# Ichoran/dbce-video-cpp

Measured on AMD Instinct MI355X. Metric: frames/s + raw-pixel GB/s, 4096x3072 U8 encode+decode round-trip, higher is better.
Workload: dtype u8

## Files before the change

### dbde-video-cpp_amd/csrc/dbde_kernels.hip

```cpp
#include "dbde_kernels.h"

#include "dbde_bits.h"
#include "dbde_device.h"


namespace dbde {

#ifndef DBDE_DIAG_LATE
#define DBDE_DIAG_LATE 34
#endif
#ifdef DBDE_DIAG
#define SF_DECL uint64_t sfd[10] = {0, 0, 0, 0, 0, 0, 0, 0, 0, 0}
#define SF_MARK(i) do { if (threadIdx.x == 0) sfd[i] = wall_clock64(); } while (0)
#define SF_DRAIN() asm volatile("s_waitcnt vmcnt(0) lgkmcnt(0)" ::: "memory")
#define SF_FLUSH(diag, last)                                                                          \
    do {                                                                                              \
        if (threadIdx.x == 0 && (diag)) {                                                             \
            atomicMax(&(diag)[0], ~(unsigned long long)sfd[0]);                                       \
            for (int i_ = 1; i_ < 10; i_++) atomicAdd(&(diag)[i_], (unsigned long long)sfd[i_]);      \
            atomicAdd(&(diag)[10], 1ull);                                                             \
            atomicMax(&(diag)[11], (unsigned long long)sfd[last]);                                    \
            atomicMax(&(diag)[12], (unsigned long long)sfd[0]);                                       \
            atomicAdd(&(diag)[13], (unsigned long long)sfd[0]);                                       \
        }                                                                                             \
    } while (0)
#else
#define SF_DECL
#define SF_MARK(i)
#define SF_DRAIN()
#define SF_FLUSH(diag, last)
#endif

typedef uint32_t u32x4_t __attribute__((ext_vector_type(4)));

typedef unsigned long long u64a;


__device__ __forceinline__ uint64_t load_u64_any(const uint8_t *p) {
    uint64_t v;
    __builtin_memcpy(&v, p, 8);
    return v;
}
__device__ __forceinline__ void store_u64_any(uint8_t *p, uint64_t v) { __builtin_memcpy(p, &v, 8); }
__device__ __forceinline__ void store_u32_bytes(uint8_t *p, uint32_t v) {
    p[0] = (uint8_t)v; p[1] = (uint8_t)(v >> 8); p[2] = (uint8_t)(v >> 16); p[3] = (uint8_t)(v >> 24);
}
__device__ __forceinline__ uint32_t load_u32_bytes(const uint8_t *p) {
    return (uint32_t)p[0] | ((uint32_t)p[1] << 8) | ((uint32_t)p[2] << 16) | ((uint32_t)p[3] << 24);
}
__device__ __forceinline__ uint64_t load_u64_bytes(const uint8_t *p) {
    return (uint64_t)load_u32_bytes(p) | ((uint64_t)load_u32_bytes(p + 4) << 32);
}

template <int NW = 4>
__device__ __forceinline__ uint32_t block_scan_incl(uint32_t v, uint32_t *s_wave_tot, int lane, int wave,
                                                    uint32_t &block_total) {
    uint32_t incl = v;
#pragma unroll
    for (int o = 1; o < 64; o <<= 1) {
        uint32_t n = __shfl_up(incl, o, 64);
        if (lane >= o) incl += n;
    }
    if (lane == 63) s_wave_tot[wave] = incl;
    __syncthreads();
    uint32_t base = 0, tot = 0;
#pragma unroll
    for (int k = 0; k < NW; k++) {
        const uint32_t tk = s_wave_tot[k];
        base += k < wave ? tk : 0u;
        tot += tk;
    }
    block_total = tot;
    return base + incl;
}

__device__ __forceinline__ uint32_t swz8(uint32_t slot) { return slot ^ ((slot >> 3) & 7u); }
__device__ __forceinline__ uint32_t swz16(uint32_t slot) { return slot ^ ((slot >> 4) & 15u); }
__device__ __forceinline__ uint32_t swzq8(uint32_t q) { return (swz8(q >> 1) << 1) | (q & 1u); }
__device__ __forceinline__ uint32_t swzq16(uint32_t q) { return (swz16(q >> 1) << 1) | (q & 1u); }

__device__ __forceinline__ uint32_t depth_bytes_bad(uint32_t x, uint32_t min_bytes) {
    return min_bytes == 1u ? ((x & 0xF0F0F0F0u) | (((x & 0x0F0F0F0Fu) + 0x77777777u) & 0x80808080u))
                           : ((x & 0xE0E0E0E0u) | (((x & 0x1F1F1F1Fu) + 0x6F6F6F6Fu) & 0x80808080u));
}

__device__ __forceinline__ uint64_t f64_to_u64_x86(double v) {
    const double two63 = 9223372036854775808.0;
    bool high = v >= two63;
    double a = high ? v - two63 : v;
    uint64_t r;
    if (a >= -two63 && a < two63) r = (uint64_t)(long long)a;
    else r = 0x8000000000000000ull;
    return high ? (r ^ 0x8000000000000000ull) : r;
}

__device__ __forceinline__ bool in_extent(uint64_t off, uint64_t len, uint64_t extent) {
    return off <= extent && len <= extent - off;
}

__device__ __forceinline__ uint32_t div_magic(uint32_t n, uint32_t d, uint32_t m, uint32_t &rem) {
    uint32_t q = __umulhi(n, m);
    uint32_t r = n - q * d;
    const bool fix = r >= d;
    q += fix ? 1u : 0u;
    r -= fix ? d : 0u;
    rem = r;
    return q;
}


__device__ __forceinline__ void load_tile_generic(const uint8_t *img, int W, int H, uint32_t w, uint32_t t,
                                                  uint32_t (&v)[16]) {
    uint32_t ty = t / w, tx = t - ty * w;
    int x0 = 8 * (int)tx;
    int rm = W - x0 < 8 ? W - x0 : 8;
#pragma unroll
    for (int r = 0; r < 8; r++) {
        int yy = 8 * (int)ty + r;
        yy = yy < H ? yy : H - 1;
        const uint8_t *row = img + (size_t)yy * (size_t)W + x0;
        uint64_t q;
        if (rm == 8) {
            q = load_u64_any(row);
        } else if (W >= 8) {
            q = load_u64_any(row + rm - 8) >> (8 * (8 - rm));
            const uint64_t last = (q >> (8 * (rm - 1))) & 0xFFull;
            q |= (last * 0x0101010101010101ull) << (8 * rm);
        } else {
            q = 0;
#pragma unroll
            for (int k = 0; k < 8; k++) {
                int kk = k < rm ? k : rm - 1;
                q |= (uint64_t)row[kk] << (8 * k);
            }
        }
        v[2 * r] = (uint32_t)q;
        v[2 * r + 1] = (uint32_t)(q >> 32);
    }
}

template <bool ALIGNED_OUT, int PIX = 1>
__device__ __forceinline__ void write_frame_fields(const EncParams &p, uint32_t f, uint32_t cf, uint32_t inf_incl,
                                                     uint32_t frame_start_glob) {
    const uint64_t meta = 32ull + (uint64_t)(1 + PIX) * p.T;
    const uint64_t frame_base = p.slot_stride ? (uint64_t)f * p.slot_stride
                                              : (uint64_t)f * meta + 8ull * (uint64_t)frame_start_glob;
    uint8_t *fb = p.out + frame_base;
    if (cf == 0u) {
        const uint64_t index = p.indices ? p.indices[f] : p.first_index + f;
        const uint64_t el = p.elapsed_ns ? p.elapsed_ns[f] : 0ull;
        const uint64_t elbits = (uint64_t)__double_as_longlong(__ull2double_rn(el));
        if (ALIGNED_OUT) {
            uint32_t *h = reinterpret_cast<uint32_t *>(fb);
            h[0] = 2u;
            h[1] = (uint32_t)index; h[2] = (uint32_t)(index >> 32);
            h[3] = (uint32_t)elbits; h[4] = (uint32_t)(elbits >> 32);
// ... 1087 lines not shown
    SF_FLUSH(p.diag, 9);
#endif
}

hipError_t launch_encode_small(const EncParams &p, bool fast_in, bool aligned_out, hipStream_t s) {
    dim3 block(kEncThreads), grid(p.n_chunks);
    switch (in_mode_of(p, fast_in) * 2 + (aligned_out ? 1 : 0)) {
        case kInFast * 2 + 1: hipLaunchKernelGGL((encode_small_kernel<kInFast, true>), grid, block, 0, s, p); break;
        case kInFast * 2 + 0: hipLaunchKernelGGL((encode_small_kernel<kInFast, false>), grid, block, 0, s, p); break;
        case kInRaw * 2 + 1: hipLaunchKernelGGL((encode_small_kernel<kInRaw, true>), grid, block, 0, s, p); break;
        case kInRaw * 2 + 0: hipLaunchKernelGGL((encode_small_kernel<kInRaw, false>), grid, block, 0, s, p); break;
        case kInBytes * 2 + 1: hipLaunchKernelGGL((encode_small_kernel<kInBytes, true>), grid, block, 0, s, p); break;
        case kInRaw4 * 2 + 1: hipLaunchKernelGGL((encode_small_kernel<kInRaw4, true>), grid, block, 0, s, p); break;
        case kInRaw4 * 2 + 0: hipLaunchKernelGGL((encode_small_kernel<kInRaw4, false>), grid, block, 0, s, p); break;
        case kInRow * 2 + 1: hipLaunchKernelGGL((encode_small_kernel<kInRow, true>), grid, block, 0, s, p); break;
        case kInRow * 2 + 0: hipLaunchKernelGGL((encode_small_kernel<kInRow, false>), grid, block, 0, s, p); break;
        default: hipLaunchKernelGGL((encode_small_kernel<kInBytes, false>), grid, block, 0, s, p); break;
    }
    return hipGetLastError();
}

__global__ __launch_bounds__(256) void encode_tiny_kernel(EncParams p) {
    const uint32_t tid = threadIdx.x, lane = tid & 63u, wave = tid >> 6;
    const uint32_t T = p.T, fpw = 64u / T;
    const uint32_t fl = lane / T, t = lane - fl * T;
    const uint32_t f = (blockIdx.x * 4u + wave) * fpw + fl;
    const bool active = fl < fpw && f < p.n_chunks;
    uint32_t v[16];
#pragma unroll
    for (int i = 0; i < 16; i++) v[i] = 0;
    if (active) load_tile_generic(p.images + (size_t)f * p.frame_pixels, p.W, p.H, p.w, t, v);
    uint32_t mn, mx;
    tile_minmax(v, mn, mx);
    const uint32_t d = active ? depth_of_range(mx - mn) : 0u;
    const uint32_t incl = wave_scan_incl(d);
    const uint32_t first = fl * T;
    const uint32_t base = (uint32_t)__shfl((int)(incl - d), (int)(first < 64u ? first : 0u), 64);
    const uint32_t upto = (uint32_t)__shfl((int)incl, (int)(first + T - 1u < 64u ? first + T - 1u : 63u), 64);
    if (!active) return;
    const uint32_t prefix = incl - d - base, total = upto - base;
    uint8_t *fb = p.out + (uint64_t)f * p.slot_stride;
    fb[24u + t] = (uint8_t)d;
    fb[28u + T + t] = (uint8_t)mn;
    uint8_t *dst = fb + 32ull + 2ull * T + 8ull * prefix;
    const uint32_t mn4 = mn * 0x01010101u;
    Funnel fn;
    fn.reset();
#pragma unroll
    for (int r = 0; r < 8; r++) {
        uint64_t word;
        if (d != 0u && fn.push(pack_row(v[2 * r] - mn4, v[2 * r + 1] - mn4, d), 8u * d, word)) {
            store_u64_any(dst, word);
            dst += 8;
        }
    }
    if (t == 0u) write_frame_fields<false>(p, f, 0u, total, 0u);
}

hipError_t launch_encode_tiny(const EncParams &p, uint32_t n_frames, hipStream_t s) {
    EncParams q = p;
    q.n_chunks = n_frames;
    q.chunks_per_frame = 1u;
    const uint32_t per_wg = 4u * (64u / p.T);
    hipLaunchKernelGGL(encode_tiny_kernel, dim3((n_frames + per_wg - 1u) / per_wg), dim3(256), 0, s, q);
    return hipGetLastError();
}

template <int THREADS>
__global__ __launch_bounds__(THREADS) void encode_mid_kernel(EncParams p) {
    constexpr int NW = THREADS / 64;
    __shared__ uint32_t s_tot[NW];
    __shared__ uint32_t s_incl[THREADS];
    const uint32_t tid = threadIdx.x, lane = tid & 63u, wave = tid >> 6;
    const uint32_t T = p.T, fpw = (uint32_t)THREADS / T;
    const uint32_t fl = tid / T, t = tid - fl * T;
    const uint32_t f = blockIdx.x * fpw + fl;
    const bool active = fl < fpw && f < p.n_chunks;
    uint32_t v[16];
#pragma unroll
    for (int i = 0; i < 16; i++) v[i] = 0;
    if (active) load_tile_generic(p.images + (size_t)f * p.frame_pixels, p.W, p.H, p.w, t, v);
    uint32_t mn, mx;
    tile_minmax(v, mn, mx);
    const uint32_t d = active ? depth_of_range(mx - mn) : 0u;
    uint32_t block_total;
    const uint32_t incl = block_scan_incl<NW>(d, s_tot, (int)lane, (int)wave, block_total);
    s_incl[tid] = incl;
    __syncthreads();
    if (!active) return;
    const uint32_t first = fl * T;
    const uint32_t base = first ? s_incl[first - 1u] : 0u;
    const uint32_t prefix = incl - d - base, total = s_incl[first + T - 1u] - base;
    uint8_t *fb = p.out + (uint64_t)f * p.slot_stride;
    fb[24u + t] = (uint8_t)d;
    fb[28u + T + t] = (uint8_t)mn;
    uint8_t *dst = fb + 32ull + 2ull * T + 8ull * prefix;
    const uint32_t mn4 = mn * 0x01010101u;
    Funnel fn;
    fn.reset();
#pragma unroll
    for (int r = 0; r < 8; r++) {
        uint64_t word;
        if (d != 0u && fn.push(pack_row(v[2 * r] - mn4, v[2 * r + 1] - mn4, d), 8u * d, word)) {
            store_u64_any(dst, word);
            dst += 8;
        }
    }
    if (t == 0u) write_frame_fields<false>(p, f, 0u, total, 0u);
}

#ifndef DBDE_MID_DECODE_MAX_THREADS
#define DBDE_MID_DECODE_MAX_THREADS 256
#endif
uint32_t mid_threads_for(uint32_t T, uint32_t max_threads) {
    uint32_t best = max_threads, best_used = 0u;
    for (uint32_t th = 256u; th <= max_threads; th *= 2u) {
        if (th < T) continue;
        const uint32_t used = (th / T) * T;
        if ((uint64_t)used * best > (uint64_t)best_used * th) { best = th; best_used = used; }
    }
    return best;
}

#ifndef DBDE_MID_ENCODE_MAX_THREADS
#define DBDE_MID_ENCODE_MAX_THREADS 1024
#endif
uint32_t mid_encode_threads_for(uint32_t T) {
    return mid_threads_for(T, T <= (unsigned)DBDE_MID_ENCODE_MAX_THREADS ? (unsigned)DBDE_MID_ENCODE_MAX_THREADS : 1024u);
}
uint32_t mid_decode_threads_for(uint32_t T) {
    return mid_threads_for(T, T <= (unsigned)DBDE_MID_DECODE_MAX_THREADS ? (unsigned)DBDE_MID_DECODE_MAX_THREADS : 1024u);
}

hipError_t launch_encode_mid(const EncParams &p, uint32_t n_frames, hipStream_t s) {
    EncParams q = p;
    q.n_chunks = n_frames;
    q.chunks_per_frame = 1u;
    const uint32_t th = mid_encode_threads_for(p.T), per_wg = th / p.T;
    const dim3 grid((n_frames + per_wg - 1u) / per_wg);
    if (th == 256u) hipLaunchKernelGGL(encode_mid_kernel<256>, grid, dim3(256), 0, s, q);
    else if (th == 512u) hipLaunchKernelGGL(encode_mid_kernel<512>, grid, dim3(512), 0, s, q);
    else hipLaunchKernelGGL(encode_mid_kernel<1024>, grid, dim3(1024), 0, s, q);
    return hipGetLastError();
}

int encode_blocks_per_cu() {
    int n = 0;
    if (hipOccupancyMaxActiveBlocksPerMultiprocessor(&n, encode_kernel<kInFast, true>, kEncThreads, 0) != hipSuccess || n < 1)
        n = 1;
    return n;
}


__global__ __launch_bounds__(1024) void decode_index_kernel(IdxParams p) {
    extern __shared__ __attribute__((aligned(16))) uint32_t s_sum[];
    __shared__ uint32_t s_part[16];
    __shared__ uint32_t s_flags;

    const uint32_t f = blockIdx.x;
    const int tid = threadIdx.x, lane = tid & 63, wave = tid >> 6;
    const uint32_t T = p.T, cpf = p.chunks_per_frame;
    const uint64_t off = p.frame_offsets[f];
    const uint64_t meta_t = (1ull + p.min_bytes) * T;
    const uint64_t need = 32ull + meta_t;
    const bool in_range = in_extent(off, need, p.stream_bytes);
    const uint8_t *fb = p.stream + off;

    for (uint32_t k = tid; k < cpf; k += blockDim.x) s_sum[k] = 0;
    if (tid == 0) s_flags = 0;
    __syncthreads();

    uint32_t bad_depth = 0;
    if (in_range) {
        const uint8_t *darr = fb + 24;
        const uint32_t head = (uint32_t)(reinterpret_cast<uintptr_t>(darr) & 15u);
        const uint8_t *a_lo = darr - head;
        const uint32_t npieces = (head + T + 15u) >> 4;
        const bool incr = p.geom.pieces == 1u && p.geom.ct >= 16u;
        const uint32_t step = 16u * blockDim.x, q_step = incr ? step / p.geom.ct : 0u, r_step = incr ? step - q_step * p.geom.ct : 0u;
        uint32_t k_run = 0, rem_run = 0;
        bool have_run = false;
        for (uint32_t i = tid; i < npieces; i += blockDim.x) {
            uint4 q;
            if (a_lo + 16ull * (i + 1u) <= p.stream + p.stream_bytes) {
                q = *reinterpret_cast<const uint4 *>(a_lo + 16ull * i);
            } else {
                uint32_t wq[4] = {0, 0, 0, 0};
                for (uint32_t b = 0; b < 16u; b++) {
                    const uint8_t *src = a_lo + 16ull * i + b;
                    if (src < p.stream + p.stream_bytes) wq[b >> 2] |= (uint32_t)*src << (8u * (b & 3u));
                }
                q = make_uint4(wq[0], wq[1], wq[2], wq[3]);
            }
            uint32_t wv[4] = {q.x, q.y, q.z, q.w};
            const long long pos0 = 16ll * i - (long long)head;
            const uint32_t lo = pos0 < 0 ? 0u : (uint32_t)pos0;
            const uint32_t hi = pos0 + 16 > (long long)T ? T : (uint32_t)(pos0 + 16);
#pragma unroll
            for (int j = 0; j < 4; j++) {
                const long long pj = pos0 + 4 * j;
                uint32_t mask = 0xFFFFFFFFu;
                if (pj < 0) mask = (pj <= -4) ? 0u : (0xFFFFFFFFu << (8 * (int)(-pj)));
                if (pj + 4 > (long long)T) {
                    const long long keep = (long long)T - pj;
                    mask &= keep <= 0 ? 0u : (keep >= 4 ? 0xFFFFFFFFu : (0xFFFFFFFFu >> (8 * (int)(4 - keep))));
                }
                wv[j] &= mask;
                bad_depth |= depth_bytes_bad(wv[j], p.min_bytes);
            }
            uint32_t k_first, k_last;
            if (incr && pos0 >= 0) {
                if (!have_run) { k_run = lo / p.geom.ct; rem_run = lo - k_run * p.geom.ct; have_run = true; }
                k_first = k_run;
                k_last = rem_run + (hi - 1u - lo) >= p.geom.ct ? k_run + 1u : k_run;
                k_run += q_step; rem_run += r_step;
                if (rem_run >= p.geom.ct) { rem_run -= p.geom.ct; k_run++; }
            } else {
                k_first = dec_chunk_of(p.geom, lo);
                k_last = dec_chunk_of(p.geom, hi - 1u);
            }
            if (k_first == k_last || (incr && pos0 >= 0)) {
                const long long bnd = k_first == k_last ? (long long)T : (long long)(k_first + 1u) * p.geom.ct;
                uint32_t sum_lo = 0, sum_hi = 0;
#pragma unroll
                for (int j = 0; j < 4; j++) {
                    const long long nb = bnd - (pos0 + 4 * j);
                    const uint32_t m = nb >= 4 ? 0xFFFFFFFFu : (nb <= 0 ? 0u : (0xFFFFFFFFu >> (8 * (int)(4 - nb))));
                    sum_lo += __builtin_amdgcn_sad_u8(wv[j] & m, 0u, 0u);
                    sum_hi += __builtin_amdgcn_sad_u8(wv[j] & ~m, 0u, 0u);
                }
                if (sum_lo) atomicAdd(&s_sum[k_first], sum_lo);
                if (sum_hi) atomicAdd(&s_sum[k_first + 1u], sum_hi);
            } else {
                for (uint32_t pos = lo; pos < hi; pos++) {
                    const uint32_t b = (uint32_t)((long long)pos - pos0);
                    const uint32_t v = (wv[b >> 2] >> (8u * (b & 3u))) & 0xFFu;
                    if (v) atomicAdd(&s_sum[dec_chunk_of(p.geom, pos)], v);
                }
            }
        }
    }
    if (bad_depth) atomicOr(&s_flags, 1u);
    __syncthreads();

    const uint32_t seg = (cpf + blockDim.x - 1u) / blockDim.x;
    const uint32_t k0 = (uint32_t)tid * seg;
    uint32_t local = 0;
    for (uint32_t k = k0; k < k0 + seg && k < cpf; k++) local += s_sum[k];
    uint32_t incl = local;
#pragma unroll
    for (int o = 1; o < 64; o <<= 1) {
        uint32_t n = __shfl_up(incl, o, 64);
        if (lane >= o) incl += n;
    }
    if (lane == 63) s_part[wave] = incl;
    __syncthreads();
    uint32_t base = 0, total = 0;
    for (int k = 0; k < (int)(blockDim.x >> 6); k++) {
        const uint32_t v = s_part[k];
        if (k < wave) base += v;
        total += v;
    }
    uint32_t run = base + incl - local;
    uint32_t *co = p.chunk_off + (size_t)f * (cpf + 1u);
    for (uint32_t k = k0; k < k0 + seg && k < cpf; k++) {
        co[k] = run;
        run += s_sum[k];
    }
    if (tid == 0) co[cpf] = total;

    if (tid == 0) {
        bool ok = in_range;
        uint32_t field = 0;
        uint64_t index = 0, elapsed = 0, consumed = 20;
        if (in_extent(off, 20, p.stream_bytes)) {
            field = load_u32_bytes(fb);
            index = load_u64_bytes(fb + 4);
            elapsed = f64_to_u64_x86(__longlong_as_double((long long)load_u64_bytes(fb + 12)));
        }
        if (ok) {
            const int32_t nb = (int32_t)load_u32_bytes(fb + 20);
            const int32_t nm = (int32_t)load_u32_bytes(fb + 24 + T);
            const int32_t n64 = (int32_t)load_u32_bytes(fb + 28 + meta_t);
            ok = nb == (int32_t)T && nm == (int32_t)(T * p.min_bytes) && n64 == (int32_t)total && !(s_flags & 1u);
            if (ok && !in_extent(off, need + 8ull * total, p.stream_bytes)) ok = false;
            if (ok) consumed = need + 8ull * total;
        }
        p.frame_ok[f] = ok ? 1u : 0u;
        if (p.results) {
            FrameResultDev *r = reinterpret_cast<FrameResultDev *>(p.results) + f;
            r->u64s = (field == 2u && ok) ? 2u : 0xFFFFFFFFu;
            r->pad_ = 0;
            r->index = index;
            r->elapsed_ns = elapsed;
            r->consumed = consumed;
        }
    }
}

__global__ __launch_bounds__(256) void decode_index_split_kernel(IdxParams p) {
    __shared__ uint32_t s_part[4];
    __shared__ uint32_t s_last;

    const uint32_t f = blockIdx.x / p.split, piece = blockIdx.x - f * p.split;
    const int tid = threadIdx.x, lane = tid & 63, wave = tid >> 6;
    const uint32_t T = p.T, cpf = p.chunks_per_frame;
    const uint64_t off = p.frame_offsets[f];
    const uint64_t meta_t = (1ull + p.min_bytes) * T;
    const uint64_t need = 32ull + meta_t;
    const bool in_range = in_extent(off, need, p.stream_bytes);
    const uint8_t *fb = p.stream + off;
    uint32_t *co = p.chunk_off + (size_t)f * (cpf + 1u);

    const uint32_t per = (cpf + p.split - 1u) / p.split;
    const uint32_t k_begin = piece * per, k_end = k_begin + per < cpf ? k_begin + per : cpf;
    uint32_t bad = 0;
    for (uint32_t k = k_begin + (uint32_t)wave; k < k_end; k += 4u) {
        uint32_t sum = 0;
        if (in_range) {
            const uint8_t *darr = fb + 24;
            const uint32_t c_lo = dec_chunk_begin(p.geom, k), c_hi = dec_chunk_begin(p.geom, k + 1u);
#pragma unroll
            for (uint32_t j = 0; j < 8u; j += 4u) {
                const uint32_t q = c_lo + (uint32_t)lane * 8u + j;
                if (q < c_hi) {
                    uint32_t x;
                    __builtin_memcpy(&x, darr + q, 4);
                    const uint32_t keep = c_hi - q;
                    if (keep < 4u) x &= 0xFFFFFFFFu >> (8u * (4u - keep));
                    bad |= depth_bytes_bad(x, p.min_bytes);
                    sum += __builtin_amdgcn_sad_u8(x, 0u, 0u);
                }
            }
        }
        const uint32_t tot = wave_scan_incl(sum);
        if (lane == 63) __hip_atomic_store(&co[k], tot, __ATOMIC_RELAXED, __HIP_MEMORY_SCOPE_AGENT);
    }
    if (__any((int)(bad != 0u)) && lane == 0) atomicOr(&p.frame_flag[f], 1u);

    asm volatile("s_waitcnt vmcnt(0)" ::: "memory");
    __syncthreads();
    if (tid == 0) s_last = atomicAdd(&p.frame_ctr[f], 1u) == p.split - 1u ? 1u : 0u;
    __syncthreads();
    if (!s_last) return;

    const uint32_t seg = (cpf + 255u) / 256u;
    const uint32_t k0 = (uint32_t)tid * seg;
    uint32_t local = 0;
    for (uint32_t k = k0; k < k0 + seg && k < cpf; k++)
        local += __hip_atomic_load(&co[k], __ATOMIC_RELAXED, __HIP_MEMORY_SCOPE_AGENT);
    const uint32_t incl = wave_scan_incl(local);
    if (lane == 63) s_part[wave] = incl;
    __syncthreads();
    uint32_t base = 0, total = 0;
#pragma unroll
    for (int k = 0; k < 4; k++) {
        const uint32_t v = s_part[k];
        base += k < wave ? v : 0u;
        total += v;
    }
    uint32_t run = base + incl - local;
    for (uint32_t k = k0; k < k0 + seg && k < cpf; k++) {
        const uint32_t v = __hip_atomic_load(&co[k], __ATOMIC_RELAXED, __HIP_MEMORY_SCOPE_AGENT);
        co[k] = run;
        run += v;
    }
    if (tid == 0) {
        co[cpf] = total;
        const uint32_t flags = __hip_atomic_load(&p.frame_flag[f], __ATOMIC_RELAXED, __HIP_MEMORY_SCOPE_AGENT);
        p.frame_flag[f] = 0;
        p.frame_ctr[f] = 0;
        bool ok = in_range;
        uint32_t field = 0;
        uint64_t index = 0, elapsed = 0, consumed = 20;
        if (in_extent(off, 20, p.stream_bytes)) {
            field = load_u32_bytes(fb);
            index = load_u64_bytes(fb + 4);
            elapsed = f64_to_u64_x86(__longlong_as_double((long long)load_u64_bytes(fb + 12)));
        }
        if (ok) {
            const int32_t nb = (int32_t)load_u32_bytes(fb + 20);
            const int32_t nm = (int32_t)load_u32_bytes(fb + 24 + T);
            const int32_t n64 = (int32_t)load_u32_bytes(fb + 28 + meta_t);
            ok = nb == (int32_t)T && nm == (int32_t)(T * p.min_bytes) && n64 == (int32_t)total && !(flags & 1u);
            if (ok && !in_extent(off, need + 8ull * total, p.stream_bytes)) ok = false;
            if (ok) consumed = need + 8ull * total;
        }
        p.frame_ok[f] = ok ? 1u : 0u;
        if (p.results) {
            FrameResultDev *r = reinterpret_cast<FrameResultDev *>(p.results) + f;
            r->u64s = (field == 2u && ok) ? 2u : 0xFFFFFFFFu;
            r->pad_ = 0;
            r->index = index;
            r->elapsed_ns = elapsed;
            r->consumed = consumed;
        }
    }
}

hipError_t launch_decode_index(const IdxParams &p, int n_frames, hipStream_t s) {
    const size_t lds = (size_t)p.chunks_per_frame * sizeof(uint32_t);
    if (lds > 48 * 1024) {
        hipError_t e = hipFuncSetAttribute(reinterpret_cast<const void *>(decode_index_kernel),
                                           hipFuncAttributeMaxDynamicSharedMemorySize, (int)lds);
        if (e != hipSuccess) return e;
    }
    if (p.split > 1u) {
        hipLaunchKernelGGL(decode_index_split_kernel, dim3((uint32_t)n_frames * p.split), dim3(256), 0, s, p);
        return hipGetLastError();
    }
    const uint32_t pieces = (p.T + 15u) / 16u + 1u;
    uint32_t threads = (pieces + 63u) / 64u * 64u;
    threads = threads < 64u ? 64u : (threads > 1024u ? 1024u : threads);
    hipLaunchKernelGGL(decode_index_kernel, dim3(n_frames), dim3(threads), lds, s, p);
    return hipGetLastError();
}

__device__ __forceinline__ uint32_t swz_byte16(uint32_t A) { return A ^ ((A >> 4) & 0xF0u); }

__device__ __forceinline__ void put_byte1(uint32_t &x, uint32_t sh, uint32_t g) {
    asm("v_lshrrev_b32_sdwa %0, %1, %2 dst_sel:BYTE_1 dst_unused:UNUSED_PRESERVE src0_sel:DWORD src1_sel:DWORD" : "+v"(x) : "v"(sh), "v"(g));
}
__device__ __forceinline__ void put_byte2(uint32_t &x, uint32_t sh, uint32_t g) {
    asm("v_lshrrev_b32_sdwa %0, %1, %2 dst_sel:BYTE_2 dst_unused:UNUSED_PRESERVE src0_sel:DWORD src1_sel:DWORD" : "+v"(x) : "v"(sh), "v"(g));
}
__device__ __forceinline__ void put_byte3(uint32_t &x, uint32_t sh, uint32_t g) {
    asm("v_lshrrev_b32_sdwa %0, %1, %2 dst_sel:BYTE_3 dst_unused:UNUSED_PRESERVE src0_sel:DWORD src1_sel:DWORD" : "+v"(x) : "v"(sh), "v"(g));
}

template <bool SWZ>
__device__ __forceinline__ void unpack_tile_from_lds(const uint8_t *s_img, uint32_t byte_base, uint32_t d,
                                                     uint32_t mn, uint32_t (&v)[16]) {
    const uint32_t mn4 = mn * 0x01010101u;
    const bool d8 = d >= 8u;
    uint32_t a = byte_base;
    const uint32_t md = ((1u << d) - 1u) * 0x01010101u;
    const uint32_t md7 = md & 0x7F7F7F7Fu, mdh = md & 0x80808080u;
    const uint32_t mnlo = mn4 & 0x7F7F7F7Fu, mnhi = mn4 & 0x80808080u;
    const uint32_t d2 = 2u * d, d3 = 3u * d;
#pragma unroll
    for (int r = 0; r < 8; r++) {
        uint32_t t0, t1, t2;
        if (SWZ) {
            const uint32_t A0 = a & ~7u;
            const uint2 lo = *reinterpret_cast<const uint2 *>(s_img + swz_byte16(A0));
            const uint2 hi = *reinterpret_cast<const uint2 *>(s_img + swz_byte16(A0 + 8u));
            const bool up = (a & 4u) != 0u;
            t0 = up ? lo.y : lo.x; t1 = up ? hi.x : lo.y; t2 = up ? hi.y : hi.x;
        } else {
            const uint32_t *q = reinterpret_cast<const uint32_t *>(s_img + (a & ~3u));
            t0 = q[0]; t1 = q[1]; t2 = q[2];
        }
        const uint32_t r_lo = __builtin_amdgcn_alignbyte(t1, t0, a);
        const uint32_t r_hi = __builtin_amdgcn_alignbyte(t2, t1, a);
        const uint32_t g_hi = d8 ? r_hi : __builtin_amdgcn_alignbit(r_hi, r_lo, 4u * d);
        uint32_t x = r_lo, y = g_hi;
        put_byte1(x, d, r_lo); put_byte2(x, d2, r_lo); put_byte3(x, d3, r_lo);
        put_byte1(y, d, g_hi); put_byte2(y, d2, g_hi); put_byte3(y, d3, g_hi);
        v[2 * r] = (((x & md7) + mnlo) ^ (x & mdh)) ^ mnhi;
        v[2 * r + 1] = (((y & md7) + mnlo) ^ (y & mdh)) ^ mnhi;
        a += d;
    }
}

__device__ __forceinline__ void unpack_tile_d8_from_lds(const uint8_t *s_img, uint32_t byte_base, uint32_t mn,
                                                        uint32_t (&v)[16]) {
    const uint32_t mn4 = mn * 0x01010101u;
#pragma unroll
    for (int r = 0; r < 8; r++) {
        const uint2 q = *reinterpret_cast<const uint2 *>(s_img + swz_byte16(byte_base + 8u * (uint32_t)r));
        v[2 * r] = add_bytes(q.x, mn4);
        v[2 * r + 1] = add_bytes(q.y, mn4);
    }
}

constexpr uint32_t kXcdRun = 16;
__device__ __forceinline__ uint32_t xcd_local_chunk(uint32_t b, uint32_t n_chunks) {
    constexpr uint32_t kGroup = 8u * kXcdRun;
    const uint32_t grp = b / kGroup, rem = b % kGroup;
    if ((grp + 1u) * kGroup > n_chunks) return b;
    return grp * kGroup + (rem & 7u) * kXcdRun + (rem >> 3);
}

template <int THREADS = 256>
struct DecLds {
    static constexpr int kThreads = THREADS;
    static constexpr int kWaves = THREADS / 64;
    static constexpr uint32_t kSlots = THREADS == 256 ? 2128u : 1600u;
    static constexpr int kPieces = (kSlots + kThreads - 1) / kThreads;
};

__device__ __forceinline__ void lds_store_u64_any(uint8_t *s_base, uint32_t byte_addr, uint32_t lo, uint32_t hi) {
    const uint64_t v = ((uint64_t)hi << 32) | lo;
    const uint32_t a = (uint32_t)(uintptr_t)(__attribute__((address_space(3))) uint8_t *)s_base + byte_addr;
    asm volatile("ds_write_b64 %0, %1" ::"v"(a), "v"(v) : "memory");
}
__device__ __forceinline__ void lds_store_bytes(uint8_t *s_px, uint32_t a, uint64_t v, uint32_t n) {
    if (n & 4u) { __builtin_memcpy(s_px + a, &v, 4); a += 4u; v >>= 32; }
    if (n & 2u) { s_px[a] = (uint8_t)v; s_px[a + 1u] = (uint8_t)(v >> 8); a += 2u; v >>= 16; }
    if (n & 1u) s_px[a] = (uint8_t)v;
}

__device__ __forceinline__ void store_tile_generic(uint8_t *img, int W, int H, uint32_t w, uint32_t t,
                                                   const uint32_t (&v)[16]) {
    uint32_t ty = t / w, tx = t - ty * w;
    int x0 = 8 * (int)tx;
    int rm = W - x0 < 8 ? W - x0 : 8;
#pragma unroll
    for (int r = 0; r < 8; r++) {
        int yy = 8 * (int)ty + r;
        if (yy < H) {
            uint8_t *row = img + (size_t)yy * (size_t)W + x0;
            const uint64_t q = ((uint64_t)v[2 * r + 1] << 32) | v[2 * r];
            if (rm == 8) {
                store_u64_any(row, q);
            } else {
#pragma unroll
                for (int k = 0; k < 8; k++)
                    if (k < rm) row[k] = (uint8_t)(q >> (8 * k));
            }
        }
    }
}

constexpr int kImgDirect = 0, kImgLinear = 1, kImgTiles = 2;

constexpr int kIdxTable = 0, kIdxSelf = 1, kIdxFused = 2;

template <int IMG, int INDEX, int THREADS = 256>
__global__ __launch_bounds__(THREADS) void decode_kernel(DecParams p) {
    constexpr bool SELF_INDEX = INDEX == kIdxSelf;
    typedef DecLds<THREADS> G;
    __shared__ __attribute__((aligned(16))) uint64_t s_in[G::kSlots * 2];
    __shared__ uint32_t s_wave_tot[G::kWaves];
    __shared__ uint32_t s_idx[G::kWaves][4];

    const int tid = threadIdx.x, lane = tid & 63, wave = tid >> 6;
    SF_DECL;
    SF_MARK(0);
    const uint32_t c = SELF_INDEX ? blockIdx.x : xcd_local_chunk(blockIdx.x, p.n_chunks);
    const uint32_t f = c / p.chunks_per_frame;
    const uint32_t cf = c - f * p.chunks_per_frame;
    const uint64_t foff = p.frame_offsets[f];
    const uint8_t *fb = p.stream + foff;
    const uint32_t t_begin = dec_chunk_begin(p.geom, cf);
    const uint32_t n_tiles = dec_chunk_begin(p.geom, cf + 1u) - t_begin;
    uint32_t w_begin, w_end;
    if (SELF_INDEX) {
        const uint32_t T = p.T;
        const uint64_t need = 32ull + 2ull * T;
        const bool in_range = in_extent(foff, need, p.stream_bytes);
        uint32_t s_before = 0, s_mine = 0, s_all = 0, bad = 0;
        if (in_range) {
            const uint8_t *darr = fb + 24;
            const uint32_t head = (uint32_t)(reinterpret_cast<uintptr_t>(darr) & 15u);
            const uint8_t *a_lo = darr - head;
            const uint32_t npieces = (head + T + 15u) >> 4;
            const uint8_t *s_end = p.stream + p.stream_bytes;
            auto account = [&](uint32_t i, const uint4 &qv) {
                const uint32_t wv[4] = {qv.x, qv.y, qv.z, qv.w};
                const int pos0 = (int)(16u * i) - (int)head;
#pragma unroll
                for (int j = 0; j < 4; j++) {
                    const int pj = pos0 + 4 * j;
                    auto below = [&](int limit) -> uint32_t {
                        const int n = limit - pj;
                        return n >= 4 ? 0xFFFFFFFFu : (n <= 0 ? 0u : (0xFFFFFFFFu >> (8 * (4 - n))));
// ... 1256 lines not shown
```

Measured before the change: 122,700.

## Batch index-kernel loads several pieces per thread with smaller workgroups

```diff
diff --git a/dbde-video-cpp_amd/csrc/dbde_index_launch.h b/dbde-video-cpp_amd/csrc/dbde_index_launch.h
--- /dev/null
+++ b/dbde-video-cpp_amd/csrc/dbde_index_launch.h
@@ -0,0 +1,46 @@
+#pragma once
+#include <stdint.h>
+
+namespace dbde {
+
+#ifndef DBDE_IDX_MAX_THREADS
+#define DBDE_IDX_MAX_THREADS 512
+#endif
+#ifndef DBDE_IDX_DEEP
+#define DBDE_IDX_DEEP 8
+#endif
+constexpr uint32_t kIdxMaxThreads = DBDE_IDX_MAX_THREADS;
+constexpr uint32_t kIdxShallow = 4;
+constexpr uint32_t kIdxDeep = DBDE_IDX_DEEP;
+static_assert(kIdxMaxThreads % 64u == 0u && kIdxMaxThreads >= 64u && kIdxMaxThreads <= 1024u, "whole waves, one workgroup");
+static_assert(kIdxDeep % 4u == 0u && kIdxDeep > kIdxShallow, "batches are held four pieces at a time");
+constexpr uint32_t kIdxMaxDynLds = 160 * 1024;
+constexpr uint32_t kIdxDefaultDynLds = 48 * 1024;
+
+struct IndexLaunch {
+    uint32_t threads;
+    uint32_t depth;
+    uint32_t batches;
+    uint32_t lds_bytes;
+    bool raise_lds;
+    uint64_t grid;
+};
+
+inline uint32_t index_pieces_for(uint32_t T) { return (T + 15u) / 16u + 1u; }
+
+inline IndexLaunch index_launch_for(uint32_t T, uint32_t cpf, uint64_t n_frames) {
+    IndexLaunch l;
+    const uint32_t pieces = index_pieces_for(T);
+    l.depth = pieces <= kIdxShallow * kIdxMaxThreads ? kIdxShallow : kIdxDeep;
+    const uint32_t per_batch_max = l.depth * kIdxMaxThreads;
+    l.batches = (pieces + per_batch_max - 1u) / per_batch_max;
+    const uint32_t per_thread = l.depth * l.batches;
+    const uint32_t need = (pieces + per_thread - 1u) / per_thread;
+    l.threads = (need + 63u) / 64u * 64u;
+    l.lds_bytes = cpf * (uint32_t)sizeof(uint32_t);
+    l.raise_lds = l.lds_bytes > kIdxDefaultDynLds;
+    l.grid = n_frames;
+    return l;
+}
+
+}
diff --git a/dbde-video-cpp_amd/csrc/dbde_kernels.hip b/dbde-video-cpp_amd/csrc/dbde_kernels.hip
--- a/dbde-video-cpp_amd/csrc/dbde_kernels.hip
+++ b/dbde-video-cpp_amd/csrc/dbde_kernels.hip
@@ -2,6 +2,7 @@
 
 #include "dbde_bits.h"
 #include "dbde_device.h"
+#include "dbde_index_launch.h"
 
 
 namespace dbde {
@@ -1395,98 +1396,149 @@
 }
 
 
-__global__ __launch_bounds__(1024) void decode_index_kernel(IdxParams p) {
+struct IdxRun {
+    bool incr, have;
+    uint32_t q_step, r_step, k, rem;
+};
+
+__device__ __forceinline__ uint32_t index_reduce_piece(const IdxParams &p, uint32_t *s_sum, const u32x4_t q, uint32_t i,
+                                                       uint32_t head, IdxRun &run, bool walk) {
+    const uint32_t T = p.T;
+    uint32_t wv[4] = {q.x, q.y, q.z, q.w};
+    uint32_t bad_depth = 0;
+    const int pos0 = 16 * (int)i - (int)head;
+    const uint32_t lo = pos0 < 0 ? 0u : (uint32_t)pos0;
+    const uint32_t hi = pos0 + 16 > (int)T ? T : (uint32_t)(pos0 + 16);
+#pragma unroll
+    for (int j = 0; j < 4; j++) {
+        const int pj = pos0 + 4 * j;
+        uint32_t mask = 0xFFFFFFFFu;
+        if (pj < 0) mask = (pj <= -4) ? 0u : (0xFFFFFFFFu << (8 * -pj));
+        if (pj + 4 > (int)T) {
+            const int keep = (int)T - pj;
+            mask &= keep <= 0 ? 0u : (keep >= 4 ? 0xFFFFFFFFu : (0xFFFFFFFFu >> (8 * (4 - keep))));
+        }
+        wv[j] &= mask;
+        bad_depth |= depth_bytes_bad(wv[j], p.min_bytes);
+    }
+    const bool incr = walk && run.incr && pos0 >= 0;
+    uint32_t k_first, k_last;
+    if (incr) {
+        if (!run.have) { run.k = lo / p.geom.ct; run.rem = lo - run.k * p.geom.ct; run.have = true; }
+        k_first = run.k;
+        k_last = run.rem + (hi - 1u - lo) >= p.geom.ct ? run.k + 1u : run.k;
+        run.k += run.q_step; run.rem += run.r_step;
+        if (run.rem >= p.geom.ct) { run.rem -= p.geom.ct; run.k++; }
+    } else {
+        k_first = dec_chunk_of(p.geom, lo);
+        k_last = dec_chunk_of(p.geom, hi - 1u);
+    }
+    if (k_first == k_last || incr) {
+        const int bnd = k_first == k_last ? (int)T : (int)((k_first + 1u) * p.geom.ct);
+        uint32_t sum_lo = 0, sum_hi = 0;
+#pragma unroll
+        for (int j = 0; j < 4; j++) {
+            const int nb = bnd - (pos0 + 4 * j);
+            const uint32_t m = nb >= 4 ? 0xFFFFFFFFu : (nb <= 0 ? 0u : (0xFFFFFFFFu >> (8 * (4 - nb))));
+            sum_lo += __builtin_amdgcn_sad_u8(wv[j] & m, 0u, 0u);
+            sum_hi += __builtin_amdgcn_sad_u8(wv[j] & ~m, 0u, 0u);
+        }
+        if (sum_lo) atomicAdd(&s_sum[k_first], sum_lo);
+        if (sum_hi) atomicAdd(&s_sum[k_first + 1u], sum_hi);
+    } else {
+        for (uint32_t pos = lo; pos < hi; pos++) {
+            const uint32_t b = (uint32_t)((int)pos - pos0);
+            const uint32_t v = (wv[b >> 2] >> (8u * (b & 3u))) & 0xFFu;
+            if (v) atomicAdd(&s_sum[dec_chunk_of(p.geom, pos)], v);
+        }
+    }
+    return bad_depth;
+}
+
+template <int D>
+__global__ __launch_bounds__(kIdxMaxThreads, 4) void decode_index_kernel(IdxParams p) {
     extern __shared__ __attribute__((aligned(16))) uint32_t s_sum[];
-    __shared__ uint32_t s_part[16];
+    __shared__ uint32_t s_part[kIdxMaxThreads / 64u];
     __shared__ uint32_t s_flags;
 
     const uint32_t f = blockIdx.x;
+    const uint32_t nthr = blockDim.x;
     const int tid = threadIdx.x, lane = tid & 63, wave = tid >> 6;
     const uint32_t T = p.T, cpf = p.chunks_per_frame;
     const uint64_t off = p.frame_offsets[f];
     const uint64_t meta_t = (1ull + p.min_bytes) * T;
     const uint64_t need = 32ull + meta_t;
     const bool in_range = in_extent(off, need, p.stream_bytes);
+    const bool head_in = in_extent(off, 20, p.stream_bytes);
     const uint8_t *fb = p.stream + off;
-
-    for (uint32_t k = tid; k < cpf; k += blockDim.x) s_sum[k] = 0;
+    const uint8_t *s_end = p.stream + p.stream_bytes;
+
+    for (uint32_t k = tid; k < cpf; k += nthr) s_sum[k] = 0;
     if (tid == 0) s_flags = 0;
-    __syncthreads();
+
+    u32x4_t h_lo = {0u, 0u, 0u, 0u};
+    uint32_t h_el_hi = 0, f_nb = 0, f_nm = 0, f_n64 = 0;
+    if (tid == 0) {
+        if (head_in) {
+            __builtin_memcpy(&h_lo, fb, 16);
+            __builtin_memcpy(&h_el_hi, fb + 16, 4);
+        }
+        if (in_range) {
+            f_nb = load_u32_bytes(fb + 20);
+            f_nm = load_u32_bytes(fb + 24 + T);
+            f_n64 = load_u32_bytes(fb + 28 + meta_t);
+        }
+    }
+
+    const uint8_t *darr = fb + 24;
+    const uint32_t head = (uint32_t)(reinterpret_cast<uintptr_t>(darr) & 15u);
+    const uint8_t *a_lo = darr - head;
+    const uint32_t npieces = in_range ? (head + T + 15u) >> 4 : 0u;
+    const uint32_t n_full = npieces != 0u && a_lo + 16ull * npieces > s_end ? npieces - 1u : npieces;
+
+    IdxRun run;
+    run.incr = p.geom.pieces == 1u && p.geom.ct >= 16u;
+    run.have = false;
+    const uint32_t step = 16u * nthr;
+    run.q_step = run.incr ? step / p.geom.ct : 0u;
+    run.r_step = run.incr ? step - run.q_step * p.geom.ct : 0u;
+    run.k = 0; run.rem = 0;
 
     uint32_t bad_depth = 0;
-    if (in_range) {
-        const uint8_t *darr = fb + 24;
-        const uint32_t head = (uint32_t)(reinterpret_cast<uintptr_t>(darr) & 15u);
-        const uint8_t *a_lo = darr - head;
-        const uint32_t npieces = (head + T + 15u) >> 4;
-        const bool incr = p.geom.pieces == 1u && p.geom.ct >= 16u;
-        const uint32_t step = 16u * blockDim.x, q_step = incr ? step / p.geom.ct : 0u, r_step = incr ? step - q_step * p.geom.ct : 0u;
-        uint32_t k_run = 0, rem_run = 0;
-        bool have_run = false;
-        for (uint32_t i = tid; i < npieces; i += blockDim.x) {
-            uint4 q;
-            if (a_lo + 16ull * (i + 1u) <= p.stream + p.stream_bytes) {
-                q = *reinterpret_cast<const uint4 *>(a_lo + 16ull * i);
-            } else {
-                uint32_t wq[4] = {0, 0, 0, 0};
-                for (uint32_t b = 0; b < 16u; b++) {
-                    const uint8_t *src = a_lo + 16ull * i + b;
-                    if (src < p.stream + p.stream_bytes) wq[b >> 2] |= (uint32_t)*src << (8u * (b & 3u));
-                }
-                q = make_uint4(wq[0], wq[1], wq[2], wq[3]);
-            }
-            uint32_t wv[4] = {q.x, q.y, q.z, q.w};
-            const long long pos0 = 16ll * i - (long long)head;
-            const uint32_t lo = pos0 < 0 ? 0u : (uint32_t)pos0;
-            const uint32_t hi = pos0 + 16 > (long long)T ? T : (uint32_t)(pos0 + 16);
-#pragma unroll
-            for (int j = 0; j < 4; j++) {
-                const long long pj = pos0 + 4 * j;
-                uint32_t mask = 0xFFFFFFFFu;
-                if (pj < 0) mask = (pj <= -4) ? 0u : (0xFFFFFFFFu << (8 * (int)(-pj)));
-                if (pj + 4 > (long long)T) {
-                    const long long keep = (long long)T - pj;
-                    mask &= keep <= 0 ? 0u : (keep >= 4 ? 0xFFFFFFFFu : (0xFFFFFFFFu >> (8 * (int)(4 - keep))));
-                }
-                wv[j] &= mask;
-                bad_depth |= depth_bytes_bad(wv[j], p.min_bytes);
-            }
-            uint32_t k_first, k_last;
-            if (incr && pos0 >= 0) {
-                if (!have_run) { k_run = lo / p.geom.ct; rem_run = lo - k_run * p.geom.ct; have_run = true; }
-                k_first = k_run;
-                k_last = rem_run + (hi - 1u - lo) >= p.geom.ct ? k_run + 1u : k_run;
-                k_run += q_step; rem_run += r_step;
-                if (rem_run >= p.geom.ct) { rem_run -= p.geom.ct; k_run++; }
-            } else {
-                k_first = dec_chunk_of(p.geom, lo);
-                k_last = dec_chunk_of(p.geom, hi - 1u);
-            }
-            if (k_first == k_last || (incr && pos0 >= 0)) {
-                const long long bnd = k_first == k_last ? (long long)T : (long long)(k_first + 1u) * p.geom.ct;
-                uint32_t sum_lo = 0, sum_hi = 0;
-#pragma unroll
-                for (int j = 0; j < 4; j++) {
-                    const long long nb = bnd - (pos0 + 4 * j);
-                    const uint32_t m = nb >= 4 ? 0xFFFFFFFFu : (nb <= 0 ? 0u : (0xFFFFFFFFu >> (8 * (int)(4 - nb))));
-                    sum_lo += __builtin_amdgcn_sad_u8(wv[j] & m, 0u, 0u);
-                    sum_hi += __builtin_amdgcn_sad_u8(wv[j] & ~m, 0u, 0u);
-                }
-                if (sum_lo) atomicAdd(&s_sum[k_first], sum_lo);
-                if (sum_hi) atomicAdd(&s_sum[k_first + 1u], sum_hi);
-            } else {
-                for (uint32_t pos = lo; pos < hi; pos++) {
-                    const uint32_t b = (uint32_t)((long long)pos - pos0);
-                    const uint32_t v = (wv[b >> 2] >> (8u * (b & 3u))) & 0xFFu;
-                    if (v) atomicAdd(&s_sum[dec_chunk_of(p.geom, pos)], v);
-                }
-            }
-        }
-    }
+    for (uint32_t base = 0; base < n_full; base += (uint32_t)D * nthr) {
+        u32x4_t q[D];
+#pragma unroll
+        for (int j = 0; j < D; j++) {
+            const uint32_t i = base + (uint32_t)j * nthr + (uint32_t)tid;
+            const uint32_t ii = i < n_full ? i : n_full - 1u;
+            q[j] = *reinterpret_cast<const u32x4_t *>(a_lo + 16ull * ii);
+        }
+        if (base == 0u) lds_barrier();
+#pragma unroll
+        for (int j = 0; j < D; j += 4)
+            asm volatile("" : "+v"(q[j]), "+v"(q[j + 1]), "+v"(q[j + 2]), "+v"(q[j + 3]) :: "memory");
+#pragma unroll
+        for (int j = 0; j < D; j++) {
+            const uint32_t i = base + (uint32_t)j * nthr + (uint32_t)tid;
+            if (i < n_full) bad_depth |= index_reduce_piece(p, s_sum, q[j], i, head, run, true);
+        }
+    }
+    if (n_full == 0u) lds_barrier();
+    if (n_full < npieces && tid == 0) {
+        const uint32_t i = npieces - 1u;
+        uint32_t wq[4] = {0, 0, 0, 0};
+        for (uint32_t b = 0; b < 16u; b++) {
+            const uint8_t *src = a_lo + 16ull * i + b;
+            if (src < s_end) wq[b >> 2] |= (uint32_t)*src << (8u * (b & 3u));
+        }
+        const u32x4_t qb = {wq[0], wq[1], wq[2], wq[3]};
+        bad_depth |= index_reduce_piece(p, s_sum, qb, i, head, run, false);
+    }
+    asm volatile("" : "+v"(h_lo), "+v"(h_el_hi), "+v"(f_nb), "+v"(f_nm), "+v"(f_n64));
     if (bad_depth) atomicOr(&s_flags, 1u);
     __syncthreads();
 
-    const uint32_t seg = (cpf + blockDim.x - 1u) / blockDim.x;
+    const uint32_t seg = (cpf + nthr - 1u) / nthr;
     const uint32_t k0 = (uint32_t)tid * seg;
     uint32_t local = 0;
     for (uint32_t k = k0; k < k0 + seg && k < cpf; k++) local += s_sum[k];
@@ -1499,16 +1551,16 @@
     if (lane == 63) s_part[wave] = incl;
     __syncthreads();
     uint32_t base = 0, total = 0;
-    for (int k = 0; k < (int)(blockDim.x >> 6); k++) {
+    for (int k = 0; k < (int)(nthr >> 6); k++) {
         const uint32_t v = s_part[k];
         if (k < wave) base += v;
         total += v;
     }
-    uint32_t run = base + incl - local;
+    uint32_t excl = base + incl - local;
     uint32_t *co = p.chunk_off + (size_t)f * (cpf + 1u);
     for (uint32_t k = k0; k < k0 + seg && k < cpf; k++) {
-        co[k] = run;
-        run += s_sum[k];
+        co[k] = excl;
+        excl += s_sum[k];
     }
     if (tid == 0) co[cpf] = total;
 
@@ -1516,15 +1568,13 @@
         bool ok = in_range;
         uint32_t field = 0;
         uint64_t index = 0, elapsed = 0, consumed = 20;
-        if (in_extent(off, 20, p.stream_bytes)) {
-            field = load_u32_bytes(fb);
-            index = load_u64_bytes(fb + 4);
-            elapsed = f64_to_u64_x86(__longlong_as_double((long long)load_u64_bytes(fb + 12)));
+        if (head_in) {
+            field = h_lo.x;
+            index = (uint64_t)h_lo.y | ((uint64_t)h_lo.z << 32);
+            elapsed = f64_to_u64_x86(__longlong_as_double((long long)((uint64_t)h_lo.w | ((uint64_t)h_el_hi << 32))));
         }
         if (ok) {
-            const int32_t nb = (int32_t)load_u32_bytes(fb + 20);
-            const int32_t nm = (int32_t)load_u32_bytes(fb + 24 + T);
-            const int32_t n64 = (int32_t)load_u32_bytes(fb + 28 + meta_t);
+            const int32_t nb = (int32_t)f_nb, nm = (int32_t)f_nm, n64 = (int32_t)f_n64;
             ok = nb == (int32_t)T && nm == (int32_t)(T * p.min_bytes) && n64 == (int32_t)total && !(s_flags & 1u);
             if (ok && !in_extent(off, need + 8ull * total, p.stream_bytes)) ok = false;
             if (ok) consumed = need + 8ull * total;
@@ -1642,20 +1692,21 @@
 }
 
 hipError_t launch_decode_index(const IdxParams &p, int n_frames, hipStream_t s) {
-    const size_t lds = (size_t)p.chunks_per_frame * sizeof(uint32_t);
-    if (lds > 48 * 1024) {
-        hipError_t e = hipFuncSetAttribute(reinterpret_cast<const void *>(decode_index_kernel),
-                                           hipFuncAttributeMaxDynamicSharedMemorySize, (int)lds);
-        if (e != hipSuccess) return e;
-    }
     if (p.split > 1u) {
         hipLaunchKernelGGL(decode_index_split_kernel, dim3((uint32_t)n_frames * p.split), dim3(256), 0, s, p);
         return hipGetLastError();
     }
-    const uint32_t pieces = (p.T + 15u) / 16u + 1u;
-    uint32_t threads = (pieces + 63u) / 64u * 64u;
-    threads = threads < 64u ? 64u : (threads > 1024u ? 1024u : threads);
-    hipLaunchKernelGGL(decode_index_kernel, dim3(n_frames), dim3(threads), lds, s, p);
+    const IndexLaunch l = index_launch_for(p.T, p.chunks_per_frame, (uint64_t)n_frames);
+    const void *fn = l.depth == kIdxShallow ? reinterpret_cast<const void *>(decode_index_kernel<(int)kIdxShallow>)
+                                            : reinterpret_cast<const void *>(decode_index_kernel<(int)kIdxDeep>);
+    if (l.raise_lds) {
+        hipError_t e = hipFuncSetAttribute(fn, hipFuncAttributeMaxDynamicSharedMemorySize, (int)l.lds_bytes);
+        if (e != hipSuccess) return e;
+    }
+    if (l.depth == kIdxShallow)
+        hipLaunchKernelGGL(decode_index_kernel<(int)kIdxShallow>, dim3((uint32_t)l.grid), dim3(l.threads), l.lds_bytes, s, p);
+    else
+        hipLaunchKernelGGL(decode_index_kernel<(int)kIdxDeep>, dim3((uint32_t)l.grid), dim3(l.threads), l.lds_bytes, s, p);
     return hipGetLastError();
 }
 
```

After: 122,000. Within noise of the previous version (-0.6%).
